# endiqq/Multi-Feature-ViT

Measured on AMD Instinct MI355X. Metric: images/sec (two-stream 224^2 vit_small MF-CA train step), higher is better.
Workload: dtype bf16x3 (split bf16 hi+lo operands, 3 MFMAs per product, f32 accumulate)

## Files before the change

### multi-feature-vit_amd/csrc/gemm_pp.hip

```cpp
#include "kernels.h"
#include "prof.h"

#include <stdlib.h>

#include <type_traits>

namespace mfvit {

namespace {

constexpr int PP_BM = 256, PP_BN = 128;
constexpr int PP_SROW = 128;
constexpr int PP_A = PP_BM * PP_SROW, PP_W = PP_BN * PP_SROW;
constexpr int PP_SLOT = PP_A + PP_W;
constexpr int PP_NSLOT = 3, PP_AHEAD = 2;
constexpr int PP_RING = PP_NSLOT * PP_SLOT;
constexpr int PP_PATCH = 16 * 128;
constexpr int PP_LDS = PP_RING + 8 * PP_PATCH;
constexpr int PP_NDA = 4, PP_NDW = 2, PP_NDMA = PP_NDA + PP_NDW;

template <int N> __device__ __forceinline__ void pp_wait_vm() { asm volatile("s_waitcnt vmcnt(%0)" ::"n"(N) : "memory"); }
__device__ __forceinline__ void pp_glds16(unsigned voff, const char* sbase, unsigned lds_dst) {
    unsigned keep;
    asm volatile("s_mov_b32 %0, m0\n\ts_mov_b32 m0, %3\n\ts_nop 0\n\tglobal_load_lds_dwordx4 %1, %2\n\ts_mov_b32 m0, %0"
                 : "=&s"(keep)
                 : "v"(voff), "s"(sbase), "s"(lds_dst)
                 : "memory");
}

typedef unsigned int pp_u32x4 __attribute__((ext_vector_type(4)));
__device__ __forceinline__ void pp_gload16(pp_u32x4& dst, const char* sbase, unsigned voff) { asm volatile("global_load_dwordx4 %0, %1, %2" : "=&v"(dst) : "v"(voff), "s"(sbase) : "memory"); }
__device__ __forceinline__ void pp_gload4(float& dst, const char* sbase, unsigned voff) { asm volatile("global_load_dword %0, %1, %2" : "=&v"(dst) : "v"(voff), "s"(sbase) : "memory"); }
__device__ __forceinline__ void pp_landed(pp_u32x4& r) { asm volatile("" : "+v"(r)); }
__device__ __forceinline__ void pp_landed(float& r) { asm volatile("" : "+v"(r)); }

template <typename T> struct PpMma;
template <> struct PpMma<sbf16> { static __device__ __forceinline__ f32x4 mma(bf16x8 a, bf16x8 b, f32x4 c) { return __builtin_amdgcn_mfma_f32_16x16x32_bf16(a, b, c, 0, 0, 0); } };
template <> struct PpMma<bf16> { static __device__ __forceinline__ f32x4 mma(bf16x8 a, bf16x8 b, f32x4 c) { return __builtin_amdgcn_mfma_f32_16x16x32_bf16(a, b, c, 0, 0, 0); } };
template <> struct PpMma<f16> { static __device__ __forceinline__ f32x4 mma(f16x8 a, f16x8 b, f32x4 c) { return __builtin_amdgcn_mfma_f32_16x16x32_f16(a, b, c, 0, 0, 0); } };

template <typename E> __device__ __forceinline__ unsigned pp_pk2(float a, float b) {
    typedef float f2 __attribute__((ext_vector_type(2)));
    typedef E e2 __attribute__((ext_vector_type(2)));
    const f2 x = {a, b};
    return __builtin_bit_cast(unsigned, __builtin_convertvector(x, e2));
}
template <typename E> __device__ __forceinline__ uint2 pp_pack4(f32x4 v) { return make_uint2(pp_pk2<E>(v[0], v[1]), pp_pk2<E>(v[2], v[3])); }
template <typename E> __device__ __forceinline__ void pp_split4(f32x4 v, uint2& hi, uint2& lo) {
    typedef float f2 __attribute__((ext_vector_type(2)));
    typedef E e2 __attribute__((ext_vector_type(2)));
    const f2 x0 = {v[0], v[1]}, x1 = {v[2], v[3]};
    const e2 h0 = __builtin_convertvector(x0, e2), h1 = __builtin_convertvector(x1, e2);
    const e2 l0 = __builtin_convertvector(x0 - __builtin_convertvector(h0, f2), e2), l1 = __builtin_convertvector(x1 - __builtin_convertvector(h1, f2), e2);
    hi = make_uint2(__builtin_bit_cast(unsigned, h0), __builtin_bit_cast(unsigned, h1));
    lo = make_uint2(__builtin_bit_cast(unsigned, l0), __builtin_bit_cast(unsigned, l1));
}

template <typename T, int EPI>
__global__ __launch_bounds__(512, 1) void gemm_nt_pp_kernel(GemmP p, int ntiles, int ntall) {
    constexpr bool SPLIT = is_split<T>::value;
    constexpr int NMF = SPLIT ? 48 : 32;
    constexpr int KPS = SPLIT ? 32 : 64;
    typedef typename Vec8<T>::type frag_t;
    typedef typename Vec4<T>::elem E16;
    typedef typename act_grad_type<T>::type AX;
    typedef pp_u32x4 u32x4;
    constexpr bool GELU = EPI == EPI_BIAS_GELU || EPI == EPI_BIAS_GELU_DROP;
    constexpr bool ACT = GELU || EPI == EPI_BIAS_RELU;
    constexpr bool HAS_BIAS = EPI == EPI_BIAS || ACT || EPI == EPI_BIAS_X3F16;
    constexpr bool SWAP = EPI != EPI_GELU_BWD;
    constexpr int NSTORE = SPLIT ? 12 : 6;
    extern __shared__ __attribute__((aligned(16))) char lds[];
    const int tid = threadIdx.x, lane = tid & 63, l15 = lane & 15, q4 = lane >> 4;
    const int wave = __builtin_amdgcn_readfirstlane(tid >> 6);
    const int grp = wave >> 2, wq = wave & 3, wm = wq >> 1, wn = wq & 1;
    const int ntn = p.N / PP_BN;
    const int nst = p.K / KPS;
    const unsigned lda_b = (unsigned)p.lda * 2u, ldw_b = (unsigned)p.ldw * 2u;
    const unsigned lbase = __builtin_amdgcn_readfirstlane((unsigned)(size_t)(__attribute__((address_space(3))) char*)lds);
    const int G = gridDim.x;
    const int my = xcd_remap(blockIdx.x, G);
    const int ntl = my < ntiles ? (ntiles - my + G - 1) / G : 0;
    if (ntl == 0) return;
    auto tile_rt = [&](int tile) { return tile / ntn; };
    auto tile_m0 = [&](int rt) { return rt < ntall ? rt * PP_BM : ntall * PP_BM + (rt - ntall) * (3 * PP_BM / 4); };
    const char* gA = (const char*)p.A;
    const char* gW = (const char*)p.W;

    unsigned va[PP_NDA], vw[PP_NDW];
    int ld_t = 0, ld_s = 0, ld_slot = 0;
    auto set_tile_offsets = [&](int t) {
        int ln = tid & 63;
        asm volatile("" : "+v"(ln));
        const int tile = my + t * G;
        const int rt = tile_rt(tile), m0 = tile_m0(rt), n0 = (tile % ntn) * PP_BN;
        const bool tall = rt < ntall;
#pragma unroll
        for (int i = 0; i < PP_NDA; ++i) {
            const int row = 8 * (wave + 8 * i) + (ln >> 3);
            const int rb = row & 63;
            int gm = tall ? m0 + row : m0 + (row >> 6) * 48 + (rb < 48 ? rb : 47);
            gm = gm < p.M ? gm : p.M - 1;
            va[i] = (unsigned)gm * lda_b + 16u * (unsigned)((ln & 7) ^ ((row >> 1) & 7));
        }
#pragma unroll
        for (int i = 0; i < PP_NDW; ++i) {
            const int row = 8 * (wave + 8 * i) + (ln >> 3);
            vw[i] = (unsigned)(n0 + row) * ldw_b + 16u * (unsigned)((ln & 7) ^ ((row >> 1) & 7));
        }
    };
    set_tile_offsets(0);
    unsigned dma_soff = 0, dma_dst = 0;
    auto dma_piece = [&](int d) __attribute__((always_inline)) {
        if (d < PP_NDA) pp_glds16(va[d], gA + dma_soff, dma_dst + d * 8 * 1024);
        else pp_glds16(vw[d - PP_NDA], gW + dma_soff, dma_dst + PP_A + (d - PP_NDA) * 8 * 1024);
    };
    auto dma_begin = [&]() __attribute__((always_inline)) {
        dma_soff = (unsigned)ld_s * PP_SROW;
        dma_dst = lbase + (unsigned)ld_slot * PP_SLOT + (unsigned)wave * 1024u;
#pragma unroll
        for (int d = 0; d < PP_NDMA; ++d) dma_piece(d);
    };
    auto dma_end = [&]() __attribute__((always_inline)) {
        ld_slot = ld_slot == PP_NSLOT - 1 ? 0 : ld_slot + 1;
        if (++ld_s == nst) {
            ld_s = 0;
            if (ld_t + 1 < ntl) { ++ld_t; set_tile_offsets(ld_t); }
        }
    };
    auto dma_stage = [&]() {
        dma_begin();
        dma_end();
    };
    unsigned fa[4], fw[4];
#pragma unroll
    for (int i = 0; i < 4; ++i) {
        const int ra = grp * 128 + wm * 64 + i * 16 + l15, rw = wn * 64 + i * 16 + l15;
        fa[i] = (unsigned)(ra * PP_SROW + 16 * (q4 ^ ((ra >> 1) & 7)));
        fw[i] = (unsigned)(PP_A + rw * PP_SROW + 16 * (q4 ^ ((rw >> 1) & 7)));
    }
    char* patch = lds + PP_RING + wave * PP_PATCH;

    constexpr int E1 = EPI == EPI_GELU_BWD ? 8 : (HAS_BIAS ? 4 : 0);
    constexpr int KEEP = PP_NDMA * (PP_AHEAD - 1);
    u32x4 bn[4];
    u32x4 ax[4][2];
    auto bias_loads = [&](int t) __attribute__((always_inline)) {
        const int tile = my + (t < ntl ? t : ntl - 1) * G;
        const unsigned nq = (unsigned)((tile % ntn) * PP_BN + wn * 64);
        const char* bsrc = p.bias ? (const char*)p.bias : (const char*)p.W;
        int lq = tid >> 4 & 3;
        asm volatile("" : "+v"(lq));
#pragma unroll
        for (int jt = 0; jt < 4; ++jt) pp_gload16(bn[jt], bsrc, (nq + jt * 16 + 4 * lq) * 4u);
    };
    if constexpr (SWAP && HAS_BIAS) bias_loads(0);
#pragma unroll
    for (int d = 0; d < PP_AHEAD; ++d) dma_stage();
    pp_wait_vm<PP_NDMA*(PP_AHEAD - 1)>();
    if constexpr (SWAP && HAS_BIAS) {
#pragma unroll
        for (int jt = 0; jt < 4; ++jt) pp_landed(bn[jt]);
    }
    __builtin_amdgcn_s_barrier();
    if (grp == 1) __builtin_amdgcn_s_barrier();
    int slot = 0;
    frag_t af[2][4], bf[2][4];
    for (int t = 0; t < ntl; ++t) {
      const int tile = my + t * G;
      auto run_tile = [&](auto mi_c) __attribute__((always_inline)) {
        constexpr int MI = decltype(mi_c)::value;
        constexpr int NMFI = NMF / 4 * MI;
        f32x4 acc[4][4];
#pragma unroll
        for (int i = 0; i < MI; ++i)
#pragma unroll
            for (int j = 0; j < 4; ++j) {
                if constexpr (SWAP && HAS_BIAS) acc[i][j] = p.bias ? __builtin_bit_cast(f32x4, bn[j]) : f32x4{0.f, 0.f, 0.f, 0.f};
                else acc[i][j] = f32x4{0.f, 0.f, 0.f, 0.f};
            }
        const int mw = tile_m0(tile_rt(tile)) + (grp * 2 + wm) * (16 * MI);
        const int nw = (tile % ntn) * PP_BN + wn * 64;
        auto stage = [&](auto last_c, bool behind_epilogue) __attribute__((always_inline)) {
            constexpr bool LAST = decltype(last_c)::value;
            const char* sl = lds + slot * PP_SLOT;
#pragma unroll
            for (int c = 0; c < 2; ++c)
#pragma unroll
                for (int i = 0; i < 4; ++i) {
                    if (i < MI) af[c][i] = *(const frag_t*)(sl + (fa[i] ^ (64u * c)));
                    bf[c][i] = *(const frag_t*)(sl + (fw[i] ^ (64u * c)));
                }
            if constexpr (LAST && EPI == EPI_GELU_BWD) {
                int ln = tid & 63;
                asm volatile("" : "+v"(ln));
#pragma unroll
                for (int u = 0; u < 4; ++u)
#pragma unroll
                    for (int q = 0; q < 2; ++q) {
                        int m = mw + (u < MI ? u : MI - 1) * 16 + 8 * q + (ln >> 3);
                        m = m < p.M ? m : p.M - 1;
                        pp_gload16(ax[u][q], (const char*)p.aux, (unsigned)m * (unsigned)(p.ldaux * (long)sizeof(AX)) + (unsigned)(nw * (int)sizeof(AX) + 16 * (ln & 7)));
                    }
            } else if constexpr (LAST && SWAP && HAS_BIAS) {
                bias_loads(t + 1);
            }
            dma_begin();
            if constexpr (LAST) pp_wait_vm<KEEP + E1>();
            else if (behind_epilogue) pp_wait_vm<KEEP + NSTORE>();
            else pp_wait_vm<KEEP>();
            asm volatile("s_waitcnt lgkmcnt(0)" ::: "memory");
            __builtin_amdgcn_s_barrier();
            __builtin_amdgcn_s_setprio(1);
#pragma unroll
            for (int tt = 0; tt < NMFI; ++tt) {
                const int term = tt / (4 * MI), i = (tt >> 2) % MI, j = tt & 3;
                const frag_t a = af[SPLIT ? (term == 0 ? 1 : 0) : term][i], w = bf[SPLIT ? (term == 1 ? 1 : 0) : term][j];
                acc[i][j] = SWAP ? PpMma<T>::mma(w, a, acc[i][j]) : PpMma<T>::mma(a, w, acc[i][j]);
            }
            dma_end();
            __builtin_amdgcn_s_setprio(0);
            __builtin_amdgcn_s_barrier();
            slot = slot == PP_NSLOT - 1 ? 0 : slot + 1;
        };
        for (int s = 0; s < nst - 1; ++s) stage(std::false_type(), t > 0 && s == 0);
        stage(std::true_type(), false);
        if (grp == 0) __builtin_amdgcn_s_barrier();

        if constexpr (E1 > 0) {
            pp_wait_vm<PP_NDMA*(PP_AHEAD - 1)>();
            if constexpr (EPI == EPI_GELU_BWD) {
#pragma unroll
                for (int u = 0; u < 4; ++u) { pp_landed(ax[u][0]); pp_landed(ax[u][1]); }
            } else {
#pragma unroll
                for (int jt = 0; jt < 4; ++jt) pp_landed(bn[jt]);
            }
        }
        auto flush = [&](char* gcol, long ld_bytes, int row0, auto stream_c) {
#pragma unroll
            for (int q = 0; q < 2; ++q) {
                const int row = 8 * q + (lane >> 3);
                const u32x4 v = *(const u32x4*)(patch + row * 128 + 16 * (SWAP ? (lane & 7) ^ (lane >> 3) : (lane & 7)));
                int m = row0 + row;
                m = m < p.M ? m : p.M - 1;
                u32x4* gp = (u32x4*)(gcol + (long)m * ld_bytes + 16 * (lane & 7));
                if constexpr (decltype(stream_c)::value) store16_stream(gp, v);
                else *gp = v;
            }
        };
        void* out = ACT ? p.out1 : p.out0;
        const long ldo_b = (ACT ? p.ldo1 : p.ldo0) * (long)sizeof(T);
        constexpr bool STREAM = !(EPI == EPI_BIAS || EPI == EPI_BIAS_X3F16);
        if constexpr (SWAP) {
            char* prow_ = patch + l15 * 128;
            auto pslot = [&](int s4) -> uint2* { return (uint2*)(prow_ + 8 * ((4 * s4 + q4) ^ (2 * (l15 & 7)))); };
            const bool want_grad = p.out0 != nullptr;
#pragma unroll
            for (int i = 0; i < MI; ++i) {
                const int row0 = mw + i * 16;
                if constexpr (ACT) {
#pragma unroll
                    for (int j = 0; j < 4; ++j) {
                        f32x4 g, d;
#pragma unroll
                        for (int r = 0; r < 4; ++r) {
                            const float v = acc[i][j][r];
                            if constexpr (GELU) {
                                float gg, dd;
                                gelu_both_t<T>(v, gg, dd);
                                if constexpr (EPI == EPI_BIAS_GELU_DROP) {
                                    int m = row0 + l15;
                                    m = m < p.M ? m : p.M - 1;
                                    const float k = drop_mul(p.drop, (unsigned)m * (unsigned)p.N + (unsigned)(nw + 16 * j + 4 * q4 + r));
                                    gg *= k; dd *= k;
                                }
                                g[r] = gg; d[r] = dd;
                            } else {
                                g[r] = fmaxf(v, 0.f); d[r] = v > 0.f ? 1.f : 0.f;
                            }
                        }
                        acc[i][j] = g;
                        if (want_grad) *pslot(j) = pp_pack4<AX>(d);
                    }
                    if (want_grad) flush((char*)p.out0 + (long)nw * (long)sizeof(AX), p.ldo0 * (long)sizeof(AX), row0, std::true_type());
                }
                if constexpr (SPLIT) {
#pragma unroll
                    for (int jp = 0; jp < 2; ++jp) {
#pragma unroll
                        for (int jj = 0; jj < 2; ++jj) {
                            uint2 hi, lo;
                            if constexpr (EPI == EPI_BIAS_X3F16) pp_split4<f16>(acc[i][2 * jp + jj], hi, lo);
                            else pp_split4<E16>(acc[i][2 * jp + jj], hi, lo);
                            *pslot(jj) = hi;
                            *pslot(2 + jj) = lo;
                        }
                        flush((char*)out + (long)(nw + jp * 32) * 4, ldo_b, row0, std::integral_constant<bool, STREAM>());
                    }
                } else {
#pragma unroll
                    for (int j = 0; j < 4; ++j) *pslot(j) = pp_pack4<E16>(acc[i][j]);
                    flush((char*)out + (long)nw * 2, ldo_b, row0, std::integral_constant<bool, STREAM>());
                }
            }
        } else {
            float csum[4] = {0.f, 0.f, 0.f, 0.f};
#pragma unroll
            for (int i = 0; i < MI; ++i) {
#pragma unroll
                for (int q = 0; q < 2; ++q) *(u32x4*)(patch + (8 * q + (lane >> 3)) * 128 + 16 * (lane & 7)) = ax[i][q];
#pragma unroll
                for (int j = 0; j < 4; ++j)
#pragma unroll
                    for (int r = 0; r < 4; ++r) {
                        const float v = acc[i][j][r] * load_elem<AX>((const AX*)(patch + (4 * q4 + r) * 128), j * 16 + l15);
                        acc[i][j][r] = v;
                        csum[j] += mw + i * 16 + 4 * q4 + r < p.M ? v : 0.f;
                    }
            }
            if (p.cs0) {
#pragma unroll
                for (int j = 0; j < 4; ++j) {
                    float c = csum[j] + __shfl_xor(csum[j], 16, 64);
                    c += __shfl_xor(c, 32, 64);
                    if (lane < 16) {
                        if (p.cpart) p.cpart[((long)(tile / ntn) * 4 + grp * 2 + wm) * p.N + nw + j * 16 + lane] = c;
                        else atomicAdd(p.cs0 + nw + j * 16 + lane, c);
                    }
                }
            }
#pragma unroll
            for (int i = 0; i < MI; ++i) {
                const int row0 = mw + i * 16;
                if constexpr (SPLIT) {
#pragma unroll
                    for (int jp = 0; jp < 2; ++jp) {
#pragma unroll
                        for (int jj = 0; jj < 2; ++jj)
#pragma unroll
                            for (int r = 0; r < 4; r += 2)
                                store_elem_pair<T>((T*)(patch + (4 * q4 + r) * 128), (T*)(patch + (4 * q4 + r + 1) * 128), jj * 16 + l15, acc[i][2 * jp + jj][r],
                                                   acc[i][2 * jp + jj][r + 1]);
                        flush((char*)out + (long)(nw + jp * 32) * 4, ldo_b, row0, std::integral_constant<bool, STREAM>());
                    }
                } else {
#pragma unroll
                    for (int j = 0; j < 4; ++j)
#pragma unroll
                        for (int r = 0; r < 4; r += 2)
                            store_elem_pair<T>((T*)(patch + (4 * q4 + r) * 128), (T*)(patch + (4 * q4 + r + 1) * 128), j * 16 + l15, acc[i][j][r], acc[i][j][r + 1]);
                    flush((char*)out + (long)nw * 2, ldo_b, row0, std::integral_constant<bool, STREAM>());
                }
            }
        }
        if (grp == 1) __builtin_amdgcn_s_barrier();
      };
      if (tile_rt(tile) < ntall) run_tile(std::integral_constant<int, 4>());
      else run_tile(std::integral_constant<int, 3>());
    }
    if (grp == 0) __builtin_amdgcn_s_barrier();
    pp_wait_vm<0>();
}

struct PpPlan { int ntall, nrt; double load, ideal; };
static PpPlan pp_plan(int M, int ntn, int cus) {
    static int sw = INT_MIN;
    const bool mix = env_switch("MFVIT_PP_MIX", 1, sw) != 0;
    const int nt_all = (M + PP_BM - 1) / PP_BM;
    struct Key { int M, ntn, cus, mix; PpPlan plan; };
    static thread_local Key cache[8];
    static thread_local int cache_n = 0, cache_next = 0;
    for (int i = 0; i < cache_n; ++i)
        if (cache[i].M == M && cache[i].ntn == ntn && cache[i].cus == cus && cache[i].mix == (int)mix) return cache[i].plan;
    PpPlan best{nt_all, nt_all, 1e30, 0.0};
    for (int na = nt_all; na >= (mix ? 0 : nt_all); --na) {
        const int rest = M - na * PP_BM;
        const int nb = rest > 0 ? (rest + 191) / 192 : 0;
        if (na < nt_all && nb == 0) continue;
        const long ntile = (long)(na + nb) * ntn, ntall_t = (long)na * ntn;
        double worst = 0.0;
        for (int w = 0; w < cus && w < ntile; ++w) {
            const long n_all = (ntile - w + cus - 1) / cus;
            const long n_tall = ntall_t > w ? (ntall_t - w + cus - 1) / cus : 0;
            const double l = 4.0 * n_tall + 3.4 * (n_all - n_tall);
            worst = l > worst ? l : worst;
        }
        if (worst < best.load - 1e-9) best = PpPlan{na, na + nb, worst, 0.0};
    }
    best.ideal = (double)M / 64.0 * ntn / cus;
    cache[cache_next] = Key{M, ntn, cus, (int)mix, best};
    cache_next = (cache_next + 1) & 7;
    if (cache_n < 8) ++cache_n;
    return best;
}
template <typename T, int EPI> int launch_pp(const GemmP& p, hipStream_t st) {
    const PpPlan plan = pp_plan(p.M, p.N / PP_BN, device_cus());
    const int ntiles = (p.N / PP_BN) * plan.nrt;
    int grid = device_cus();
    if (grid > ntiles) grid = ntiles;
    static PerDeviceOnce attr_set;
    if (attr_set.first()) (void)hipFuncSetAttribute((const void*)gemm_nt_pp_kernel<T, EPI>, hipFuncAttributeMaxDynamicSharedMemorySize, PP_LDS);
    ProfScope ps(PROF_GEMM_TILE, 2.0 * p.M * p.N * p.K, 0, st);
    MFVIT_LAUNCH((gemm_nt_pp_kernel<T, EPI>), dim3(grid), dim3(512), PP_LDS, st, p, ntiles, plan.ntall);
    MFVIT_CHECK_LAUNCH();
    return MFVIT_OK;
}
template <typename T> int pp_by_epi(int epi, const GemmP& p, hipStream_t st) {
    switch (epi) {
        case EPI_BIAS: return launch_pp<T, EPI_BIAS>(p, st);
        case EPI_BIAS_GELU: return launch_pp<T, EPI_BIAS_GELU>(p, st);
        case EPI_BIAS_GELU_DROP: return launch_pp<T, EPI_BIAS_GELU_DROP>(p, st);
        case EPI_GELU_BWD: return launch_pp<T, EPI_GELU_BWD>(p, st);
        case EPI_NONE: return launch_pp<T, EPI_NONE>(p, st);
        case EPI_BIAS_RELU: return launch_pp<T, EPI_BIAS_RELU>(p, st);
        case EPI_BIAS_X3F16:
            if constexpr (is_split<T>::value) return launch_pp<T, EPI_BIAS_X3F16>(p, st);
            return MFVIT_EINVAL;
    }
    return MFVIT_EINVAL;
}

}

bool gemm_nt_pp_supported(int dtype, int epi, const GemmP& p) {
    static int c_on = INT_MIN;
    const int on = env_switch("MFVIT_PP", 1, c_on);
    if (!on) return false;
    if (dtype != MFVIT_BF16X3 && dtype != MFVIT_BF16 && dtype != MFVIT_F16) return false;
    if (epi == EPI_BIAS_X3F16 && dtype != MFVIT_BF16X3) return false;
    if (epi == EPI_COL2IM16) return false;
    const int kps = dtype == MFVIT_BF16X3 ? 32 : 64;
    if (p.nb > 1 || (on != 2 && p.M < 2048) || p.M < 1 || p.N % PP_BN || p.K % kps || p.K < 2 * kps) return false;
    if (p.omax) return false;
    if (on != 2) {
        const int cus = device_cus();
        const PpPlan plan = pp_plan(p.M, p.N / PP_BN, cus);
        if ((long)plan.nrt * (p.N / PP_BN) < cus || plan.ideal < 0.75 * plan.load) return false;
    }
    if ((p.lda * 2) % 16 || (p.ldw * 2) % 16) return false;
    if ((unsigned long long)(p.M - 1) * p.lda * 2 + 4096 >= (1ull << 32) || (unsigned long long)(p.N - 1) * p.ldw * 2 + 4096 >= (1ull << 32)) return false;
    if (epi == EPI_GELU_BWD && (!p.aux || (p.ldaux * 2) % 16 || (unsigned long long)(p.M - 1) * p.ldaux * 2 + (unsigned long long)p.N * 2 + 4096 >= (1ull << 32))) return false;
    return true;
}
int gemm_nt_pp(int dtype, int epi, const GemmP& p, hipStream_t st) {
    int rc = MFVIT_EINVAL;
    switch (dtype) {
        case MFVIT_BF16X3: rc = pp_by_epi<sbf16>(epi, p, st); break;
        case MFVIT_BF16: rc = pp_by_epi<bf16>(epi, p, st); break;
        case MFVIT_F16: rc = pp_by_epi<f16>(epi, p, st); break;
    }
    if (rc == MFVIT_OK && epi == EPI_GELU_BWD && p.cs0 && p.cpart)
        return colpart_reduce(p.cpart, 4 * pp_plan(p.M, p.N / PP_BN, device_cus()).nrt, p.N, 1, p.cs0, nullptr, nullptr, st);
    return rc;
}

}
```

Baseline: 5017.

## Route GELU-backward epilogue through swapped row-layout store path with DPP column sums

The GELU-backward GEMM epilogue now goes through the swizzled row-layout (SWAP) store path by default. The activation-gradient tile is staged in LDS using the same swizzled slot layout, multiplied into the accumulators in registers, and accumulated into per-lane column sums. Those sums are reduced across lanes with DPP and written as float4 partials (or atomics). The intent is to replace the older non-swapped column-major epilogue, which does a scalar LDS load per element and has its own reduction, with the vectorised swizzled path. An env switch keeps the old path available, and an alignment check is added for cpart.

```diff
diff --git a/multi-feature-vit_amd/csrc/gemm_pp.hip b/multi-feature-vit_amd/csrc/gemm_pp.hip
--- a/multi-feature-vit_amd/csrc/gemm_pp.hip
+++ b/multi-feature-vit_amd/csrc/gemm_pp.hip
@@ -56,7 +56,7 @@
     lo = make_uint2(__builtin_bit_cast(unsigned, l0), __builtin_bit_cast(unsigned, l1));
 }
 
-template <typename T, int EPI>
+template <typename T, int EPI, bool ROWL = true>
 __global__ __launch_bounds__(512, 1) void gemm_nt_pp_kernel(GemmP p, int ntiles, int ntall) {
     constexpr bool SPLIT = is_split<T>::value;
     constexpr int NMF = SPLIT ? 48 : 32;
@@ -68,7 +68,7 @@
     constexpr bool GELU = EPI == EPI_BIAS_GELU || EPI == EPI_BIAS_GELU_DROP;
     constexpr bool ACT = GELU || EPI == EPI_BIAS_RELU;
     constexpr bool HAS_BIAS = EPI == EPI_BIAS || ACT || EPI == EPI_BIAS_X3F16;
-    constexpr bool SWAP = EPI != EPI_GELU_BWD;
+    constexpr bool SWAP = EPI != EPI_GELU_BWD || ROWL;
     constexpr int NSTORE = SPLIT ? 12 : 6;
     extern __shared__ __attribute__((aligned(16))) char lds[];
     const int tid = threadIdx.x, lane = tid & 63, l15 = lane & 15, q4 = lane >> 4;
@@ -256,9 +256,32 @@
             char* prow_ = patch + l15 * 128;
             auto pslot = [&](int s4) -> uint2* { return (uint2*)(prow_ + 8 * ((4 * s4 + q4) ^ (2 * (l15 & 7)))); };
             const bool want_grad = p.out0 != nullptr;
+            float cs[4][4];
+            if constexpr (EPI == EPI_GELU_BWD) {
+#pragma unroll
+                for (int j = 0; j < 4; ++j)
+#pragma unroll
+                    for (int r = 0; r < 4; ++r) cs[j][r] = 0.f;
+            }
 #pragma unroll
             for (int i = 0; i < MI; ++i) {
                 const int row0 = mw + i * 16;
+                if constexpr (EPI == EPI_GELU_BWD) {
+                    typedef typename Vec4<AX>::type ax4;
+#pragma unroll
+                    for (int q = 0; q < 2; ++q) *(u32x4*)(patch + (8 * q + (lane >> 3)) * 128 + 16 * ((lane & 7) ^ (lane >> 3))) = ax[i][q];
+                    const bool live = row0 + l15 < p.M;
+#pragma unroll
+                    for (int j = 0; j < 4; ++j) {
+                        const ax4 g = __builtin_bit_cast(ax4, *pslot(j));
+#pragma unroll
+                        for (int r = 0; r < 4; ++r) {
+                            const float v = acc[i][j][r] * to_f32(g[r]);
+                            acc[i][j][r] = v;
+                            cs[j][r] += live ? v : 0.f;
+                        }
+                    }
+                }
                 if constexpr (ACT) {
 #pragma unroll
                     for (int j = 0; j < 4; ++j) {
@@ -302,6 +325,31 @@
 #pragma unroll
                     for (int j = 0; j < 4; ++j) *pslot(j) = pp_pack4<E16>(acc[i][j]);
                     flush((char*)out + (long)nw * 2, ldo_b, row0, std::integral_constant<bool, STREAM>());
+                }
+            }
+            if constexpr (EPI == EPI_GELU_BWD) {
+                if (p.cs0) {
+                    auto dpp = [](float x, auto ctrl) __attribute__((always_inline)) {
+                        return __builtin_bit_cast(float, __builtin_amdgcn_update_dpp(0, __builtin_bit_cast(int, x), decltype(ctrl)::value, 0xf, 0xf, false));
+                    };
+#pragma unroll
+                    for (int j = 0; j < 4; ++j) {
+                        float4 c4;
+#pragma unroll
+                        for (int r = 0; r < 4; ++r) {
+                            float c = cs[j][r];
+                            c += dpp(c, std::integral_constant<int, 0xB1>{});
+                            c += dpp(c, std::integral_constant<int, 0x4E>{});
+                            c += dpp(c, std::integral_constant<int, 0x141>{});
+                            c += dpp(c, std::integral_constant<int, 0x140>{});
+                            (&c4.x)[r] = c;
+                        }
+                        if (l15 == 0) {
+                            const int n = nw + j * 16 + 4 * q4;
+                            if (p.cpart) *(float4*)(p.cpart + ((long)(tile / ntn) * 4 + grp * 2 + wm) * p.N + n) = c4;
+                            else { atomicAdd(p.cs0 + n, c4.x); atomicAdd(p.cs0 + n + 1, c4.y); atomicAdd(p.cs0 + n + 2, c4.z); atomicAdd(p.cs0 + n + 3, c4.w); }
+                        }
+                    }
                 }
             }
         } else {
@@ -394,15 +442,15 @@
     if (cache_n < 8) ++cache_n;
     return best;
 }
-template <typename T, int EPI> int launch_pp(const GemmP& p, hipStream_t st) {
+template <typename T, int EPI, bool ROWL = true> int launch_pp(const GemmP& p, hipStream_t st) {
     const PpPlan plan = pp_plan(p.M, p.N / PP_BN, device_cus());
     const int ntiles = (p.N / PP_BN) * plan.nrt;
     int grid = device_cus();
     if (grid > ntiles) grid = ntiles;
     static PerDeviceOnce attr_set;
-    if (attr_set.first()) (void)hipFuncSetAttribute((const void*)gemm_nt_pp_kernel<T, EPI>, hipFuncAttributeMaxDynamicSharedMemorySize, PP_LDS);
+    if (attr_set.first()) (void)hipFuncSetAttribute((const void*)gemm_nt_pp_kernel<T, EPI, ROWL>, hipFuncAttributeMaxDynamicSharedMemorySize, PP_LDS);
     ProfScope ps(PROF_GEMM_TILE, 2.0 * p.M * p.N * p.K, 0, st);
-    MFVIT_LAUNCH((gemm_nt_pp_kernel<T, EPI>), dim3(grid), dim3(512), PP_LDS, st, p, ntiles, plan.ntall);
+    MFVIT_LAUNCH((gemm_nt_pp_kernel<T, EPI, ROWL>), dim3(grid), dim3(512), PP_LDS, st, p, ntiles, plan.ntall);
     MFVIT_CHECK_LAUNCH();
     return MFVIT_OK;
 }
@@ -411,7 +459,11 @@
         case EPI_BIAS: return launch_pp<T, EPI_BIAS>(p, st);
         case EPI_BIAS_GELU: return launch_pp<T, EPI_BIAS_GELU>(p, st);
         case EPI_BIAS_GELU_DROP: return launch_pp<T, EPI_BIAS_GELU_DROP>(p, st);
-        case EPI_GELU_BWD: return launch_pp<T, EPI_GELU_BWD>(p, st);
+        case EPI_GELU_BWD: {
+            static int sw = INT_MIN;
+            if (env_switch("MFVIT_PP_ACT_ROWL", 1, sw) == 0) return launch_pp<T, EPI_GELU_BWD, false>(p, st);
+            return launch_pp<T, EPI_GELU_BWD>(p, st);
+        }
         case EPI_NONE: return launch_pp<T, EPI_NONE>(p, st);
         case EPI_BIAS_RELU: return launch_pp<T, EPI_BIAS_RELU>(p, st);
         case EPI_BIAS_X3F16:
@@ -440,6 +492,7 @@
     }
     if ((p.lda * 2) % 16 || (p.ldw * 2) % 16) return false;
     if ((unsigned long long)(p.M - 1) * p.lda * 2 + 4096 >= (1ull << 32) || (unsigned long long)(p.N - 1) * p.ldw * 2 + 4096 >= (1ull << 32)) return false;
+    if (epi == EPI_GELU_BWD && p.cpart && ((size_t)p.cpart & 15)) return false;
     if (epi == EPI_GELU_BWD && (!p.aux || (p.ldaux * 2) % 16 || (unsigned long long)(p.M - 1) * p.ldaux * 2 + (unsigned long long)p.N * 2 + 4096 >= (1ull << 32))) return false;
     return true;
 }
```

New measurement: 5043 (median of 6 runs). About the same (+0.5%).
